# wuxiaolang/Cube_SLAM_wu

Hardware: AMD Instinct MI355X
Metric: frames/sec detect_cuboid (higher is better)
Workload: dtype f64

## Files before the change

### cube_slam_wu_amd/csrc/detect_host.cpp

```cpp
#include <hip/hip_runtime.h>

#include <algorithm>
#include <atomic>
#include <condition_variable>
#include <memory>
#include <mutex>
#include <chrono>
#include <cmath>
#include <limits>
#include <cstdio>
#include <cstring>
#include <functional>
#include <numeric>
#include <string>
#include <thread>
#include <vector>

#include "../../include/cubeslam_hip.h"
#include "detect_types.h"

namespace cs {
void launch_vp_support(const DetectDeviceView& v, const SweepParams& sp, int vp_total, hipStream_t st);
void launch_vp_support_only(const DetectDeviceView& v, const SweepParams& sp, int vp_total, hipStream_t st, int rp_max = 0);
void launch_vp_points(const DetectDeviceView& v, int vp_total, hipStream_t st);
// ... 289 lines not shown
    std::iota(keep.begin(), keep.end(), 0);
  }
  int k = (int)keep.size();
  double dmin = 1e6, dmax = -1, amin = 1e6, amax = -1;
  for (int i = 0; i < k; i++) {
    double d = dist[keep[i]], a = angle[keep[i]];
    dmin = std::min(dmin, d); dmax = std::max(dmax, d);
    amin = std::min(amin, a); amax = std::max(amax, a);
  }
  score.resize(k);
  if (k > 1) {
    bool na = (amax - amin) > 0;
    for (int i = 0; i < k; i++) {
      double d = (dist[keep[i]] - dmin) / (dmax - dmin);
      double a = angle[keep[i]];
      if (na) a = (a - amin) / (amax - amin);
      score[i] = (d + w_angle * a) / (1 + w_angle);
    }
  } else {
    for (int i = 0; i < k; i++) score[i] = (dist[keep[i]] + w_angle * angle[keep[i]]) / (1 + w_angle);
  }
}

}

struct cs_detector {
  cs_detect_params prm;
  int device = 0;
  hipStream_t stream = nullptr;
  hipStream_t stream2 = nullptr;
  hipStream_t stream3 = nullptr;
  hipStream_t stream4 = nullptr;
  hipStream_t stream_hi = nullptr;
  hipEvent_t ev[12] = {};
  int n_threads = 1;
  int cpu_grant = 1;
  std::unique_ptr<WorkerPool> pool;
  cs_batch* single = nullptr;
  std::mutex single_mu;
  void* lines_scratch = nullptr;
  void (*lines_free)(void*) = nullptr;
  void* lsd_scratch = nullptr;
  void (*lsd_free)(void*) = nullptr;
  std::mutex lines_mu;
};

struct FrameIn {
  double K[9], invK[9], R[9], t[3];
  int img_w, img_h, n_boxes, n_lines;
  std::vector<double> boxes;
  std::vector<double> lines;
  std::vector<long long> map_offs;
  std::vector<cs_roi> rois;
  std::vector<int> n_heights;
};

struct JobHost {
  int frame, box, hid;
  int yaw_off_local;
  std::vector<double> mids_x, mids_y, angs;
  std::vector<int> tops;
  int line_cap = 0;
};

struct FrameRound {
  std::vector<cs::JobDesc> jobs;
  std::vector<JobHost> jh;
  std::vector<double> yaw, yaw_c, yaw_s;
// ... 33 lines not shown
  DevBuf<unsigned long long> rp_pool_used;
  DevBuf<double> rp_raw_euler;
  PinBuf<int> h_rp_tab_count, h_rp_maps;
  PinBuf<double> h_rp_raw_euler;
  PinBuf<long long> h_rp_last_slot, h_rp_box_base;
  PinBuf<unsigned long long> h_rp_pool_used;
  long long rp_pool_cap = 0;
  int rp_NT = 0, rp_YCAP = 0;
  std::vector<hipEvent_t> rp_ev;
  bool rp_mode = false;
  PinBuf<cs::JobDesc> h_jobs_in, h_jobs_out;
  PinBuf<long long> h_slot_prefix, h_job_cbase;
  PinBuf<int> h_vp_prefix, h_top_x, h_box_job0, h_box_njobs, h_win_count, h_fallback, h_job_valid;
  PinBuf<double> h_yaw, h_yaw_c, h_yaw_s;
  PinBuf<long long> h_fb_src, h_fb_dst, h_fb_slot, h_win_slots;
  PinBuf<int> h_fb_cnt, h_fb_flag;
  PinBuf<double> h_fb_dist, h_fb_angle, h_fb_skew, h_win_corners;
  hipEvent_t done = nullptr, ev[13] = {};
  cs::DetectDeviceView view{};
  int f0 = 0, f1 = 0, vp_total = 0;
  size_t nj = 0, nb = 0;
  long long slot_total = 0;
  bool in_flight = false;
  void release() {
    jobs.release(); slot_prefix.release(); job_cbase.release(); c_slot.release(); fb_slot.release();
    vp_prefix.release(); top_x.release(); flag.release(); job_valid.release(); c_flag.release(); box_job0.release(); box_njobs.release(); win_count.release();
    fallback.release(); fb_flag.release(); mid_x.release(); mid_y.release(); ang.release(); yaw.release(); yaw_c.release(); yaw_s.release();
    vp.release(); bound.release(); bound3.release(); ls_order.release(); blk_info.release(); ls_crowded.release(); h_ls_order.release(); c_dist.release(); c_angle.release(); c_skew.release(); fb_dist.release(); fb_angle.release(); fb_skew.release();
    winners.release(); records.release(); h_records.release(); rp_trip_cnt.release(); rp_cur_idx.release(); rp_tab_count.release(); rp_maps.release(); rp_last_slot.release(); rp_box_base.release(); rp_pool_used.release(); rp_raw_euler.release(); h_rp_tab_count.release(); h_rp_maps.release(); h_rp_raw_euler.release(); h_rp_last_slot.release(); h_rp_box_base.release(); h_rp_pool_used.release(); h_jobs_in.release(); h_jobs_out.release(); h_slot_prefix.release(); h_job_cbase.release(); h_vp_prefix.release();
    h_top_x.release(); h_box_job0.release(); h_box_njobs.release(); h_win_count.release(); h_fallback.release(); h_job_valid.release(); h_yaw.release();
    h_yaw_c.release(); h_yaw_s.release();
    h_fb_src.release(); h_fb_dst.release(); h_fb_slot.release(); h_win_slots.release(); h_fb_cnt.release(); h_fb_flag.release(); h_fb_dist.release(); h_fb_angle.release();
    h_fb_skew.release(); h_win_corners.release();
    if (done) (void)hipEventDestroy(done);
    for (auto& e : ev) if (e) (void)hipEventDestroy(e);
    for (auto& e : rp_ev) if (e) (void)hipEventDestroy(e);
    rp_ev.clear();
    done = nullptr; for (auto& e : ev) e = nullptr;
  }
};

struct BatchRunState;
struct cs_batch {
  cs_detector* det = nullptr;
  BatchRunState* run_state = nullptr;
  PinBuf<cs::RpPose> h_rp;
// ... 126 lines not shown
void** cs_internal_detector_lines_slot(cs_detector* d, void (*deleter)(void*)) { d->lines_free = deleter; return &d->lines_scratch; }
void** cs_internal_detector_lsd_slot(cs_detector* d, void (*deleter)(void*)) { d->lsd_free = deleter; return &d->lsd_scratch; }
void* cs_internal_detector_lines_mutex(cs_detector* d) { return (void*)&d->lines_mu; }
void cs_internal_detector_parallel(cs_detector* d, int n, void (*fn)(int, void*), void* ctx) { d->pool->run(n, [&](int i) { fn(i, ctx); }); }
void cs_internal_detector_parallel_long(cs_detector* d, int n, void (*fn)(int, void*), void* ctx) { d->pool->run(n, [&](int i) { fn(i, ctx); }, 2 * d->cpu_grant + 1); }
int cs_internal_detector_device(cs_detector* d) { return d->device; }

int cs_detector_create(const cs_detect_params* params, int device, cs_detector** out) {
  if (!out) return CS_ERR_INVALID_ARG;
  *out = nullptr;
  int n = 0;
  if (hipGetDeviceCount(&n) != hipSuccess || n <= 0) {
    set_err("no HIP device visible; libcubeslam_hip has no CPU fallback");
    return CS_ERR_NO_DEVICE;
  }
  if (device < 0 || device >= n) { set_err("device index out of range"); return CS_ERR_INVALID_ARG; }
  CS_GUARD_BEGIN
  struct Guard { cs_detector* d; ~Guard() { if (d) cs_detector_destroy(d); } } g{new cs_detector()};
  cs_detector* d = g.d;
  if (params) d->prm = *params; else cs_detect_default_params(&d->prm);
  if (d->prm.max_cuboid_num < 1 || !(d->prm.yaw_step_deg > 0) || !(d->prm.yaw_range_deg >= 0)) { set_err("bad params"); return CS_ERR_INVALID_ARG; }
  d->device = device;
  HIP_TRY(hipSetDevice(device));
  HIP_TRY(hipStreamCreateWithFlags(&d->stream, hipStreamNonBlocking));
  HIP_TRY(hipStreamCreateWithFlags(&d->stream2, hipStreamNonBlocking));
  HIP_TRY(hipStreamCreateWithFlags(&d->stream3, hipStreamNonBlocking));
  HIP_TRY(hipStreamCreateWithFlags(&d->stream4, hipStreamNonBlocking));
  {
    int prio_low = 0, prio_high = 0;
    HIP_TRY(hipDeviceGetStreamPriorityRange(&prio_low, &prio_high));
    HIP_TRY(hipStreamCreateWithPriority(&d->stream_hi, hipStreamNonBlocking, prio_high));
  }
  for (auto& e : d->ev) HIP_TRY(hipEventCreate(&e));
  int hc = (int)std::thread::hardware_concurrency();
  int dflt = std::max(1, std::min(hc, 64));
  d->cpu_grant = std::max(1, hc);
  if (FILE* fq = std::fopen("/sys/fs/cgroup/cpu.max", "r")) {
    long long quota = 0, period = 0;
    if (std::fscanf(fq, "%lld %lld", &quota, &period) == 2 && quota > 0 && period > 0) {
      dflt = std::max(1, std::min(dflt, std::max(8, (int)(3 * quota / period))));
      d->cpu_grant = std::max(1, std::min(d->cpu_grant, (int)(quota / period)));
    }
    std::fclose(fq);
  }
  d->n_threads = d->prm.host_threads > 0 ? d->prm.host_threads : dflt;
  d->pool.reset(new WorkerPool(d->n_threads - 1));
  *out = d;
  g.d = nullptr;
  return CS_OK;
  CS_GUARD_END("cs_detector_create")
}

void cs_detector_destroy(cs_detector* d) {
  if (!d) return;
  (void)hipSetDevice(d->device);
  if (d->single) { cs_batch_destroy(d->single); d->single = nullptr; }
  if (d->lines_scratch && d->lines_free) { d->lines_free(d->lines_scratch); d->lines_scratch = nullptr; }
  if (d->lsd_scratch && d->lsd_free) { d->lsd_free(d->lsd_scratch); d->lsd_scratch = nullptr; }
  for (auto& e : d->ev) if (e) (void)hipEventDestroy(e);
  if (d->stream) (void)hipStreamDestroy(d->stream);
  if (d->stream2) (void)hipStreamDestroy(d->stream2);
  if (d->stream3) (void)hipStreamDestroy(d->stream3);
  if (d->stream4) (void)hipStreamDestroy(d->stream4);
  if (d->stream_hi) (void)hipStreamDestroy(d->stream_hi);
  delete d;
}

static int batch_fill(cs_detector* d, cs_batch* b, const cs_frame_desc* fr, const unsigned char* const* grays, int n_frames);
static void edge_rois_largest_first(std::vector<cs::EdgeRoi>& er) {
  if (er.size() <= 1024) return;
  std::stable_sort(er.begin(), er.end(), [](const cs::EdgeRoi& a, const cs::EdgeRoi& c) { return (long long)a.w * a.h > (long long)c.w * c.h; });
}
static int batch_layout(cs_detector* d, cs_batch* b);
static int batch_run_impl(cs_detector* d, cs_batch* b, cs_cuboid* out, int* out_counts, bool defer);
static int batch_flush_refill(cs_detector* d, cs_batch* b);
static void release_batch_buffers(cs_batch* b);
static int batch_create_impl(cs_detector* d, const cs_frame_desc* fr, const unsigned char* const* grays, int n_frames, cs_batch** out) {
  if (!d || !out || (!fr && n_frames) || n_frames < 0) return CS_ERR_INVALID_ARG;
  *out = nullptr;
  CS_GUARD_BEGIN
  HIP_TRY(hipSetDevice(d->device));
  struct Guard { cs_batch* b; ~Guard() { if (b) cs_batch_destroy(b); } } g{new cs_batch()};
  g.b->det = d;
  int rc = batch_fill(d, g.b, fr, grays, n_frames);
  if (rc) return rc;
  *out = g.b;
  g.b = nullptr;
// ... 192 lines not shown
    cs::launch_edge_maps(nxt ? b->d_gray2.p : b->d_gray.p, b->gray_w, b->gray_h, b->d_edge_rois.p, b->edge_n_rois, b->d_cls.p, b->d_maps.p, b->edge_max_w, b->edge_max_px, 80, 200, st);
    HIP_TRY(hipGetLastError());
  }
  HIP_TRY(hipEventRecord(b->ev_edge_done[nxt], st));
  b->gray_cur = nxt;
  b->refill_q[0] = b->refill_q[1]; b->refill_q[1] = -1; b->n_refill--;
  return CS_OK;
}
int cs_batch_refill_wait(cs_batch* b) {
  if (!b) return CS_ERR_INVALID_ARG;
  if (!b->copy_stream) return CS_OK;
  HIP_TRY(hipSetDevice(b->det->device));
  HIP_TRY(hipStreamSynchronize(b->copy_stream));
  return CS_OK;
}

int cs_batch_max_boxes(const cs_batch* b) { return b ? b->max_boxes : CS_ERR_INVALID_ARG; }

static void batch_drop_run_state(cs_batch* b);
void cs_batch_destroy(cs_batch* b) {
  if (!b) return;
  (void)hipSetDevice(b->det->device);
  if (b->run_state) { (void)hipDeviceSynchronize(); batch_drop_run_state(b); }
  release_batch_buffers(b);
  delete b;
}
static void release_batch_buffers(cs_batch* b) {
  b->pipe[0].release(); b->pipe[1].release();
  b->d_maps.release(); b->d_invK.release(); b->d_frame_lines.release(); b->d_frame_line_ptr.release(); b->d_jobs.release(); b->d_slot_prefix.release(); b->d_job_cbase.release();
  b->d_c_slot.release(); b->d_win_slots.release(); b->d_vp_prefix.release(); b->d_top_x.release(); b->d_flag.release();
  b->d_job_valid.release(); b->d_c_flag.release(); b->d_mid_x.release(); b->d_mid_y.release(); b->d_ang.release();
  b->d_yaw.release(); b->d_yaw_c.release(); b->d_yaw_s.release(); b->d_vp.release(); b->d_bound.release(); b->d_dist.release();
  b->d_angle.release(); b->d_skew.release(); b->d_corners.release(); b->d_c_dist.release(); b->d_c_angle.release();
  b->d_c_skew.release(); b->d_win_corners.release(); b->d_rp.release(); b->h_rp.release();
  b->d_gray.release(); b->d_cls.release(); b->d_edge_rois.release(); b->h_maps_stage.release(); b->d_gray2.release();
  if (b->copy_stream) { (void)hipStreamSynchronize(b->copy_stream); (void)hipStreamDestroy(b->copy_stream); b->copy_stream = nullptr; }
  for (auto& e : b->ev_copied) if (e) { (void)hipEventDestroy(e); e = nullptr; }
  for (auto& e : b->ev_edge_done) if (e) { (void)hipEventDestroy(e); e = nullptr; }
  b->h_stage.release(); b->h_c_slot.release(); b->h_job_cbase.release(); b->h_c_flag.release(); b->h_job_valid.release();
  b->h_c_dist.release(); b->h_c_angle.release(); b->h_c_skew.release(); b->h_win_corners.release();
  b->d_box_job0.release(); b->d_box_njobs.release(); b->d_win_count.release(); b->d_fallback.release(); b->d_winners.release(); b->d_last_slot.release(); b->h_last_slot.release();
  b->h_winners.release(); b->h_win_count.release(); b->h_fallback.release(); b->h_jobs.release(); b->h_tables.release(); b->h_tables2.release();
  b->d_fb_src.release(); b->d_fb_dst.release(); b->d_fb_slot.release(); b->d_fb_cnt.release(); b->d_fb_flag.release();
  b->d_fb_dist.release(); b->d_fb_angle.release(); b->d_fb_skew.release();
}

// ... 181 lines not shown
      for (int q = 0; q < NBK; q++) cnt[q + 1] += cnt[q];
      for (size_t j = 0; j < nj; j++) S.h_ls_order.p[cnt[bucket(S.h_jobs_in.p[j])]++] = (int)j;
    }
    if (vo > 0x7fffffffLL) { set_err("too many yaw samples in one chunk"); return CS_ERR_CAPACITY; }
  }
  S.nb = nb;
  MARK(1, tq);
  MARK(2, tq);
  C.tm->setup_host_ms += now_ms() - t0;
  C.tm->n_jobs += (long long)nj; C.tm->n_slots += real_slots;
  const long long slot_total = S.slot_total;
  PENS(S.ls_order, nj); PENS(S.jobs, nj); PENS(S.slot_prefix, nj + 1); PENS(S.vp_prefix, nj + 1); PENS(S.job_valid, nj); PENS(S.job_cbase, nj + 1);
  PENS(S.mid_x, n_lines + 1); PENS(S.mid_y, n_lines + 1); PENS(S.ang, n_lines + 1); PENS(S.yaw, n_yaw + 1); PENS(S.yaw_c, n_yaw + 1); PENS(S.yaw_s, n_yaw + 1);
  PENS(S.top_x, n_top + 1); PENS(S.vp, 6 * (size_t)S.vp_total + 6); PENS(S.bound, 6 * (size_t)S.vp_total + 6); PENS(S.bound3, nj * (size_t)cs::vp3_table_doubles_per_job());
  PENS(S.blk_info, 2 * (size_t)(slot_total >> 8) + 4); PENS(S.ls_crowded, 2 * (nj + 1) + 2);
  PENS(S.c_slot, slot_total + 1); PENS(S.c_flag, slot_total + 1); PENS(S.c_dist, slot_total + 1);
  PENS(S.c_angle, slot_total + 1); PENS(S.c_skew, slot_total + 1); PENS(S.box_job0, nb + 1); PENS(S.box_njobs, nb + 1); PENS(S.win_count, nb + 1);
  PENS(S.fallback, nb + 1); PENS(S.winners, nb * KMAX + 1); PENS(S.records, nb * KMAX + 1); PENS(S.h_records, nb * KMAX + 1);
  PENS(S.h_win_count, nb + 1); PENS(S.h_fallback, nb + 1); PENS(S.h_job_valid, nj); PENS(S.h_job_cbase, nj + 1); PENS(S.h_jobs_out, nj);
  int* p_ls_order = S.ls_order.p; cs::JobDesc* p_jobs = S.jobs.p; long long* p_slot_prefix = S.slot_prefix.p; int* p_vp_prefix = S.vp_prefix.p;
  double *p_yaw = S.yaw.p, *p_yaw_c = S.yaw_c.p, *p_yaw_s = S.yaw_s.p;
  int *p_top_x = S.top_x.p, *p_box_job0 = S.box_job0.p, *p_box_njobs = S.box_njobs.p;
  cs_cuboid* p_records = S.records.p; int *p_win_count = S.win_count.p, *p_fallback = S.fallback.p, *p_job_valid = S.job_valid.p; long long* p_job_cbase = S.job_cbase.p;
  S.merged_io = nj <= 256;
  if (S.merged_io) {
    size_t need = 0;
    auto room = [&](size_t bytes) { const size_t at = need; need += (bytes + 255) & ~(size_t)255; return at; };
    const size_t o_ls = room(sizeof(int) * nj), o_sp = room(sizeof(long long) * (nj + 1)), o_vp = room(sizeof(int) * (nj + 1));
    const size_t o_y = room(8 * n_yaw), o_yc = room(8 * n_yaw), o_ys = room(8 * n_yaw), o_tx = room(sizeof(int) * n_top), o_b0 = room(sizeof(int) * nb), o_bn = room(sizeof(int) * nb);
    const size_t o_jobs = room(sizeof(cs::JobDesc) * nj), in_end = need;
    S.o_jobs = o_jobs; S.o_rec = room(sizeof(cs_cuboid) * nb * KMAX); S.o_wc = room(sizeof(int) * nb); S.o_fb = room(sizeof(int) * nb); S.o_jv = room(sizeof(int) * nj);
    S.o_cb = room(sizeof(long long) * (nj + 1)); S.o_end = need;
    PENS(S.tab_arena, need + 256); PENS(S.h_tab_arena, need + 256);
    unsigned char *hb = S.h_tab_arena.p, *db = S.tab_arena.p;
    memcpy(hb + o_ls, S.h_ls_order.p, sizeof(int) * nj); memcpy(hb + o_jobs, S.h_jobs_in.p, sizeof(cs::JobDesc) * nj);
    memcpy(hb + o_sp, S.h_slot_prefix.p, sizeof(long long) * (nj + 1)); memcpy(hb + o_vp, S.h_vp_prefix.p, sizeof(int) * (nj + 1));
    if (n_yaw) { memcpy(hb + o_y, S.h_yaw.p, 8 * n_yaw); memcpy(hb + o_yc, S.h_yaw_c.p, 8 * n_yaw); memcpy(hb + o_ys, S.h_yaw_s.p, 8 * n_yaw); }
    if (n_top) memcpy(hb + o_tx, S.h_top_x.p, sizeof(int) * n_top);
    if (nb) { memcpy(hb + o_b0, S.h_box_job0.p, sizeof(int) * nb); memcpy(hb + o_bn, S.h_box_njobs.p, sizeof(int) * nb); }
    HIP_TRY(hipMemcpyAsync(db, hb, in_end, hipMemcpyHostToDevice, st));
    p_ls_order = reinterpret_cast<int*>(db + o_ls); p_jobs = reinterpret_cast<cs::JobDesc*>(db + o_jobs); p_slot_prefix = reinterpret_cast<long long*>(db + o_sp);
    p_vp_prefix = reinterpret_cast<int*>(db + o_vp); p_yaw = reinterpret_cast<double*>(db + o_y); p_yaw_c = reinterpret_cast<double*>(db + o_yc); p_yaw_s = reinterpret_cast<double*>(db + o_ys);
    p_top_x = reinterpret_cast<int*>(db + o_tx); p_box_job0 = reinterpret_cast<int*>(db + o_b0); p_box_njobs = reinterpret_cast<int*>(db + o_bn);
    p_records = reinterpret_cast<cs_cuboid*>(db + S.o_rec); p_win_count = reinterpret_cast<int*>(db + S.o_wc); p_fallback = reinterpret_cast<int*>(db + S.o_fb);
    p_job_valid = reinterpret_cast<int*>(db + S.o_jv); p_job_cbase = reinterpret_cast<long long*>(db + S.o_cb);
  } else {
    cs::CopySegs cp{};
    cs::add_copy(cp, S.ls_order, S.h_ls_order, nj); cs::add_copy(cp, S.jobs, S.h_jobs_in, nj); cs::add_copy(cp, S.slot_prefix, S.h_slot_prefix, nj + 1);
    cs::add_copy(cp, S.vp_prefix, S.h_vp_prefix, nj + 1); cs::add_copy(cp, S.yaw, S.h_yaw, n_yaw); cs::add_copy(cp, S.yaw_c, S.h_yaw_c, n_yaw);
    cs::add_copy(cp, S.yaw_s, S.h_yaw_s, n_yaw); cs::add_copy(cp, S.top_x, S.h_top_x, n_top); cs::add_copy(cp, S.box_job0, S.h_box_job0, nb);
    cs::add_copy(cp, S.box_njobs, S.h_box_njobs, nb);
    cs::launch_multi_copy(cp, st);
  }
  cs::DetectDeviceView& v = S.view;
  v = cs::DetectDeviceView{};
  v.jobs = p_jobs; v.n_jobs = (int)nj; v.slot_prefix = p_slot_prefix; v.vp_prefix = p_vp_prefix; v.maps = b->d_maps.p;
  v.mid_x = S.mid_x.p; v.mid_y = S.mid_y.p; v.line_angle = S.ang.p; v.yaw = p_yaw; v.yaw_cos = p_yaw_c; v.yaw_sin = p_yaw_s; v.top_x = p_top_x;
  v.rp = b->d_rp.p; v.invK = b->d_invK.p; v.vp = S.vp.p; v.bound = S.bound.p; v.bound3 = S.bound3.p; v.job_valid = p_job_valid;
  v.job_cbase = p_job_cbase; v.c_slot = S.c_slot.p; v.c_flag = S.c_flag.p; v.c_dist = S.c_dist.p; v.c_angle = S.c_angle.p; v.c_skew = S.c_skew.p;
  hipStream_t stB = d->stream2;
  HIP_TRY(hipEventRecord(S.ev[7], st));
  HIP_TRY(hipStreamWaitEvent(stB, S.ev[7], 0));
  HIP_TRY(hipEventRecord(S.ev[8], stB));
  v.blk_info = S.blk_info.p;
  HIP_TRY(hipMemsetAsync(S.blk_info.p, 0, sizeof(int), stB));
  cs::launch_candidate_compact(v, C.sp, stB);
  HIP_TRY(hipEventRecord(S.ev[9], stB));
  HIP_TRY(hipEventRecord(S.ev[10], stB));
  HIP_TRY(hipEventRecord(S.ev[0], st));
  cs::launch_line_setup_listed(p_jobs, (int)nj, b->d_frame_lines.p, b->d_frame_line_ptr.p, S.mid_x.p, S.mid_y.p, S.ang.p, P.pre_merge_dist_thre, P.pre_merge_angle_thre, P.edge_length_threshold, st, p_ls_order,
                               d->stream3, S.ev[0], S.ev[12], S.ls_crowded.p);
  HIP_TRY(hipEventRecord(S.ev[1], st));
  cs::launch_vp_support_only(v, C.sp, S.vp_total, st, 1);
  HIP_TRY(hipEventRecord(S.ev[2], st));
  HIP_TRY(hipStreamWaitEvent(st, S.ev[10], 0));
  HIP_TRY(hipEventRecord(S.ev[4], st));
  cs::launch_score(v, C.sp, slot_total, slot_total, st);
  HIP_TRY(hipEventRecord(S.ev[5], st));
  cs::RankView rv{};
  rv.box_job0 = p_box_job0; rv.box_njobs = p_box_njobs; rv.n_boxes = (int)nb; rv.winners = S.winners.p; rv.win_count = p_win_count; rv.fallback = p_fallback;
  cs::RankParams rkp{P.weight_vp_angle, P.weight_skew_error, P.nominal_skew_ratio, P.max_cut_skew, KMAX, C.sp.short_sq_bound};
  cs::launch_rank(v, rv, rkp, st, 0, false);
  cs::launch_records(v, rv, KMAX, p_records, st, nullptr, rkp.short_sq_bound);
  HIP_TRY(hipEventRecord(S.ev[6], st));
  HIP_TRY(hipGetLastError());
  if (S.merged_io) {
    HIP_TRY(hipMemcpyAsync(S.h_tab_arena.p + S.o_jobs, S.tab_arena.p + S.o_jobs, S.o_end - S.o_jobs, hipMemcpyDeviceToHost, st));
  } else {
    cs::CopySegs cp{};
    cs::add_copy(cp, S.h_records, S.records, nb * KMAX); cs::add_copy(cp, S.h_win_count, S.win_count, nb); cs::add_copy(cp, S.h_fallback, S.fallback, nb);
    cs::add_copy(cp, S.h_job_valid, S.job_valid, nj); cs::add_copy(cp, S.h_job_cbase, S.job_cbase, nj + 1);
    cs::launch_multi_copy(cp, st);
  }
  HIP_TRY(hipEventRecord(S.done, st));
  S.in_flight = true;
  MARK(3, tq);
  return CS_OK;
}

int pipe_finish(PipeCtx& C, PipeSlot& S, const std::vector<std::vector<CamCache>>& cam_rp) {
  cs_detector* d = C.d; cs_batch* b = C.b;
  const cs_detect_params& P = d->prm;
  const int KMAX = P.max_cuboid_num, MB = b->max_boxes;
  cs_detect_timing& tm = *C.tm;
  double tw = now_ms(), tq = tw;
  HIP_TRY(hipEventSynchronize(S.done));
  tm.d2h_ms += now_ms() - tw;
  S.in_flight = false;
  const size_t nj = S.nj, nb = S.nb;
  if (nj == 0) return CS_OK;
  if (S.merged_io) {
    const unsigned char* hb = S.h_tab_arena.p;
    memcpy(S.h_jobs_out.p, hb + S.o_jobs, sizeof(cs::JobDesc) * nj);
    if (nb) { memcpy(S.h_records.p, hb + S.o_rec, sizeof(cs_cuboid) * nb * KMAX); memcpy(S.h_win_count.p, hb + S.o_wc, sizeof(int) * nb); memcpy(S.h_fallback.p, hb + S.o_fb, sizeof(int) * nb); }
    memcpy(S.h_job_valid.p, hb + S.o_jv, sizeof(int) * nj); memcpy(S.h_job_cbase.p, hb + S.o_cb, sizeof(long long) * (nj + 1));
  }
  double t0 = now_ms();
  {
    float ms = 0;
    HIP_TRY(hipEventElapsedTime(&ms, S.ev[0], S.ev[1])); tm.line_setup_ms += ms;
    HIP_TRY(hipEventElapsedTime(&ms, S.ev[1], S.ev[2])); tm.vp_kernel_ms += ms;
    HIP_TRY(hipEventElapsedTime(&ms, S.ev[8], S.ev[9])); tm.cand_kernel_ms += ms;
    HIP_TRY(hipEventElapsedTime(&ms, S.ev[9], S.ev[10])); tm.compact_ms += ms;
    HIP_TRY(hipEventElapsedTime(&ms, S.ev[4], S.ev[5])); tm.score_kernel_ms += ms;
    HIP_TRY(hipEventElapsedTime(&ms, S.ev[5], S.ev[6])); tm.rank_kernel_ms += ms;
    tm.cand_kernel_launches += 1;
    long long n_valid = 0;
    for (size_t j = 0; j < nj; j++) n_valid += S.h_job_valid.p[j];
// ... 247 lines not shown
    slots_all += so;
  }
  const size_t nj = ji, nb = nb_tot;
  S.nj = nj; S.nb = nb; S.slot_total = slots_all; S.vp_total = vp_cap_max;
  if (n_lines > 0x7fffffffLL) { set_err("chunk too large"); return CS_ERR_CAPACITY; }
  for (size_t j = 0; j < nj; j++) S.h_ls_order.p[j] = (int)j;
  C.tm->setup_host_ms += now_ms() - t0;
  C.tm->n_jobs += (long long)nj;
  if (nj == 0) { S.in_flight = true; HIP_TRY(hipEventRecord(S.done, st)); return CS_OK; }
  PENS(S.ls_order, nj); PENS(S.jobs, nj); PENS(S.slot_prefix, nj + MB + 1); PENS(S.vp_prefix, nj + MB + 1); PENS(S.job_valid, nj); PENS(S.job_cbase, nj + MB + 1);
  const int max_trips = (int)std::min<long long>((max_job_slots + 4095) / 4096, 1 << 20);
  PENS(S.rp_trip_cnt, (size_t)nj_round_max * (size_t)std::max(1, max_trips) + 1);
  PENS(S.mid_x, (size_t)n_lines + 1); PENS(S.mid_y, (size_t)n_lines + 1); PENS(S.ang, (size_t)n_lines + 1); PENS(S.yaw, n_yaw + 1); PENS(S.yaw_c, n_yaw + 1); PENS(S.yaw_s, n_yaw + 1);
  PENS(S.top_x, n_top + 1); PENS(S.vp, 6 * (size_t)vp_cap_max + 6); PENS(S.bound, 6 * (size_t)vp_cap_max + 6); PENS(S.bound3, nj_round_max * (size_t)cs::vp3_table_doubles_per_job() + 1);
  PENS(S.flag, slot_cap_max + 1); PENS(S.c_slot, slot_cap_max + 1); PENS(S.c_flag, slot_cap_max + 1); PENS(S.c_dist, slot_cap_max + 1); PENS(S.c_angle, slot_cap_max + 1); PENS(S.c_skew, slot_cap_max + 1);
  PENS(S.box_job0, nb + 1); PENS(S.box_njobs, nb + 1); PENS(S.win_count, nb + 1); PENS(S.fallback, nb + 1); PENS(S.rp_last_slot, nb + 1);
  PENS(S.winners, nb * KMAX + 1); PENS(S.records, nb * KMAX + 1); PENS(S.h_records, nb * KMAX + 1); PENS(S.h_win_count, nb + 1); PENS(S.h_fallback, nb + 1);
  PENS(S.h_job_cbase, nj + MB + 1);
  S.rp_NT = NT; S.rp_YCAP = YCAP;
  S.rp_pool_cap = std::max<long long>(1 << 18, slots_all / 64);
  PENS(S.fb_dist, (size_t)S.rp_pool_cap + 1); PENS(S.fb_angle, (size_t)S.rp_pool_cap + 1); PENS(S.fb_skew, (size_t)S.rp_pool_cap + 1); PENS(S.fb_flag, (size_t)S.rp_pool_cap + 1); PENS(S.fb_slot, (size_t)S.rp_pool_cap + 1);
  PENS(S.ls_crowded, 2 * (nj + 1) + 2);
  PENS(S.rp_box_base, nb + 1); PENS(S.rp_pool_used, 1); PENS(S.h_rp_box_base, nb + 1); PENS(S.h_rp_pool_used, 1); PENS(S.h_rp_last_slot, nb + 1); PENS(S.h_job_valid, nj + 1); PENS(S.h_jobs_out, nj + 1);
  HIP_TRY(hipMemsetAsync(S.rp_pool_used.p, 0, sizeof(unsigned long long), st));
  PENS(S.rp_cur_idx, (size_t)NF + 1); PENS(S.rp_tab_count, (size_t)NF * NT + 1); PENS(S.rp_maps, 3 * (size_t)MB * NF + 1); PENS(S.rp_raw_euler, 3 * (size_t)NF + 1);
  {
    cs::CopySegs cp{};
    cs::add_copy(cp, S.ls_order, S.h_ls_order, nj); cs::add_copy(cp, S.jobs, S.h_jobs_in, nj); cs::add_copy(cp, S.slot_prefix, S.h_slot_prefix, nj + MB);
    cs::add_copy(cp, S.vp_prefix, S.h_vp_prefix, nj + MB); cs::add_copy(cp, S.yaw, S.h_yaw, n_yaw); cs::add_copy(cp, S.yaw_c, S.h_yaw_c, n_yaw);
    cs::add_copy(cp, S.yaw_s, S.h_yaw_s, n_yaw); cs::add_copy(cp, S.top_x, S.h_top_x, n_top); cs::add_copy(cp, S.box_job0, S.h_box_job0, nb);
    cs::add_copy(cp, S.box_njobs, S.h_box_njobs, nb); cs::add_copy(cp, S.rp_tab_count, S.h_rp_tab_count, (long long)NF * NT);
    cs::add_copy(cp, S.rp_maps, S.h_rp_maps, 3LL * MB * NF); cs::add_copy(cp, S.rp_raw_euler, S.h_rp_raw_euler, 3LL * NF);
    cs::launch_multi_copy(cp, st);
  }
  HIP_TRY(hipMemsetAsync(S.job_valid.p, 0, sizeof(int) * nj, st));
  HIP_TRY(hipMemsetAsync(S.rp_cur_idx.p, 0, sizeof(int) * NF, st));
  HIP_TRY(hipEventRecord(S.ev[0], st));
  cs::launch_line_setup_listed(S.jobs.p, (int)nj, b->d_frame_lines.p, b->d_frame_line_ptr.p, S.mid_x.p, S.mid_y.p, S.ang.p, P.pre_merge_dist_thre, P.pre_merge_angle_thre, P.edge_length_threshold, st, S.ls_order.p,
                               d->stream3, S.ev[0], S.ev[12], S.ls_crowded.p);
  HIP_TRY(hipEventRecord(S.ev[1], st));
  cs::RankParams rkp{P.weight_vp_angle, P.weight_skew_error, P.nominal_skew_ratio, P.max_cut_skew, KMAX, C.sp.short_sq_bound};
  while (S.rp_ev.size() < 5 * (size_t)MB) { hipEvent_t e = nullptr; HIP_TRY(hipEventCreate(&e)); S.rp_ev.push_back(e); }
  for (int r = 0; r < MB; r++) {
    const PipeSlot::RpRound& Rr = S.rp_rounds[r];
    if (Rr.nj == 0) continue;
    hipEvent_t* re = &S.rp_ev[5 * (size_t)r];
    cs::DetectDeviceView v{};
    v.jobs = S.jobs.p + Rr.j0; v.n_jobs = (int)Rr.nj; v.slot_prefix = S.slot_prefix.p + Rr.j0 + r; v.vp_prefix = S.vp_prefix.p + Rr.j0 + r; v.maps = b->d_maps.p;
    v.mid_x = S.mid_x.p; v.mid_y = S.mid_y.p; v.line_angle = S.ang.p; v.yaw = S.yaw.p; v.yaw_cos = S.yaw_c.p; v.yaw_sin = S.yaw_s.p; v.top_x = S.top_x.p;
    v.rp = b->d_rp.p; v.invK = b->d_invK.p; v.vp = S.vp.p; v.bound = S.bound.p; v.bound3 = S.bound3.p; v.flag = S.flag.p; v.job_valid = S.job_valid.p + Rr.j0;
    v.job_cbase = S.job_cbase.p + Rr.j0 + r; v.c_slot = S.c_slot.p; v.c_flag = S.c_flag.p; v.c_dist = S.c_dist.p; v.c_angle = S.c_angle.p; v.c_skew = S.c_skew.p;
    if (r > 0) {
      int rq = r - 1;
      while (rq > 0 && S.rp_rounds[rq].nj == 0) rq--;
      const PipeSlot::RpRound& Rq = S.rp_rounds[rq];
      cs::RpCarryView c{};
      c.n_frames = NF; c.NT = NT; c.YCAP = YCAP;
      c.prev_box_of_frame = Rq.nj ? S.rp_maps.p + (size_t)(3 * rq) * NF : nullptr;
      c.prev_last_slot = S.rp_last_slot.p + Rq.b0; c.prev_jobs = S.jobs.p + Rq.j0; c.prev_box_job0 = S.box_job0.p + Rq.b0; c.prev_box_njobs = S.box_njobs.p + Rq.b0;
      c.job0_of_frame = S.rp_maps.p + (size_t)(3 * r + 1) * NF; c.njobs_of_frame = S.rp_maps.p + (size_t)(3 * r + 2) * NF;
      c.tab_count = S.rp_tab_count.p; c.cur_idx = S.rp_cur_idx.p;
      cs::launch_rp_carry(c, S.jobs.p + Rr.j0, st);
    }
    HIP_TRY(hipEventRecord(re[0], st));
    cs::launch_vp_points(v, Rr.vp_cap, st);
// ... 8 lines not shown
    rv.box_job0 = S.box_job0.p + Rr.b0; rv.box_njobs = S.box_njobs.p + Rr.b0; rv.n_boxes = (int)Rr.nb; rv.winners = S.winners.p + Rr.b0 * KMAX;
    rv.win_count = S.win_count.p + Rr.b0; rv.fallback = S.fallback.p + Rr.b0; rv.last_slot = S.rp_last_slot.p + Rr.b0;
    cs::launch_rank(v, rv, rkp, st, Rr.nb ? (long long)(Rr.slot_cap / (long long)Rr.nb) : 0, false);
    cs::launch_records(v, rv, KMAX, S.records.p + Rr.b0 * KMAX, st, S.rp_raw_euler.p, rkp.short_sq_bound);
    {
      cs::RpSaveView sv{};
      sv.fallback = rv.fallback; sv.box_job0 = rv.box_job0; sv.box_njobs = rv.box_njobs; sv.n_boxes = rv.n_boxes; sv.pool_used = S.rp_pool_used.p; sv.pool_cap = S.rp_pool_cap;
      sv.box_base = S.rp_box_base.p + Rr.b0; sv.p_dist = S.fb_dist.p; sv.p_angle = S.fb_angle.p; sv.p_skew = S.fb_skew.p; sv.p_flag = S.fb_flag.p; sv.p_slot = S.fb_slot.p;
      cs::launch_rp_save_fallback(v, sv, st);
    }
    HIP_TRY(hipEventRecord(re[4], st));
    HIP_TRY(hipGetLastError());
  }
  HIP_TRY(hipEventRecord(S.ev[6], st));
  {
    cs::CopySegs cp{};
    cs::add_copy(cp, S.h_records, S.records, nb * KMAX); cs::add_copy(cp, S.h_win_count, S.win_count, nb); cs::add_copy(cp, S.h_fallback, S.fallback, nb);
    cs::add_copy(cp, S.h_job_cbase, S.job_cbase, nj + MB); cs::add_copy(cp, S.h_job_valid, S.job_valid, nj); cs::add_copy(cp, S.h_jobs_out, S.jobs, nj);
    cs::add_copy(cp, S.h_rp_last_slot, S.rp_last_slot, nb); cs::add_copy(cp, S.h_rp_box_base, S.rp_box_base, nb); cs::add_copy(cp, S.h_rp_pool_used, S.rp_pool_used, 1);
    cs::launch_multi_copy(cp, st);
  }
  HIP_TRY(hipEventRecord(S.done, st));
  S.in_flight = true;
  return CS_OK;
}

int rp_finish(PipeCtx& C, PipeSlot& S) {
  cs_detector* d = C.d; cs_batch* b = C.b;
  const cs_detect_params& P = d->prm;
  const int KMAX = P.max_cuboid_num, MB = b->max_boxes, NF = b->n_frames;
  cs_detect_timing& tm = *C.tm;
  double tw = now_ms();
  HIP_TRY(hipEventSynchronize(S.done));
  tm.d2h_ms += now_ms() - tw;
  S.in_flight = false;
  if (S.nj == 0) return CS_OK;
  double t0 = now_ms();
  {
    float ms = 0;
    HIP_TRY(hipEventElapsedTime(&ms, S.ev[0], S.ev[1])); tm.line_setup_ms += ms;
    for (int r = 0; r < MB; r++) {
      if (S.rp_rounds[r].nj == 0) continue;
      hipEvent_t* re = &S.rp_ev[5 * (size_t)r];
      HIP_TRY(hipEventElapsedTime(&ms, re[0], re[1])); tm.cand_kernel_ms += ms;
      HIP_TRY(hipEventElapsedTime(&ms, re[1], re[2])); tm.vp_kernel_ms += ms;
      HIP_TRY(hipEventElapsedTime(&ms, re[2], re[3])); tm.score_kernel_ms += ms;
      HIP_TRY(hipEventElapsedTime(&ms, re[3], re[4])); tm.rank_kernel_ms += ms;
      tm.cand_kernel_launches += 1;
    }
    tm.n_slots += S.slot_total;
    for (int r = 0; r < MB; r++) if (S.rp_rounds[r].nj) tm.n_valid += S.h_job_cbase.p[S.rp_rounds[r].j0 + r + S.rp_rounds[r].nj];
  }
  std::vector<char> redo(NF, 0);
  std::vector<char> host_done(S.nb, 0);
  int n_redo = 0;
// ... 951 lines not shown
```

### cube_slam_wu_amd/csrc/detect_kernels.hip

```cpp
#include <hip/hip_runtime.h>
#include "cs_hip_util.h"

#include <cstdio>
#include <cstdlib>
#include <cstring>

#include "../../include/cubeslam_hip.h"
#include "detect_types.h"

namespace cs {

__device__ __forceinline__ int wave_uniform_i32(int x) { return __builtin_amdgcn_readfirstlane(x); }
__device__ __forceinline__ long long wave_uniform_i64(long long x) {
  const unsigned lo = (unsigned)__builtin_amdgcn_readfirstlane((int)(unsigned)(x & 0xffffffffll)), hi = (unsigned)__builtin_amdgcn_readfirstlane((int)(x >> 32));
  return (long long)(((unsigned long long)hi << 32) | lo);
}
template <typename T>
__device__ __forceinline__ int find_job_wave(const T* __restrict__ prefix, int n, T elem) {
  const T first = sizeof(T) == 8 ? (T)wave_uniform_i64((long long)elem) : (T)wave_uniform_i32((int)elem);
  int lo = 0, hi = n;
  while (hi - lo > 1) {
    const int mid = (lo + hi) >> 1;
    if (prefix[mid] <= first) lo = mid; else hi = mid;
  }
// ... 1450 lines not shown
}
#else
static constexpr bool skip_kernel(const char*) { return false; }
#endif
void launch_line_setup(JobDesc* jobs, int n_jobs, const double* frame_lines, const int* frame_line_ptr, double* mid_x, double* mid_y, double* line_angle,
                       double dist_thre, double angle_thre_deg, double len_thre, hipStream_t st) {
  if (skip_kernel("line_setup")) return;
  if (n_jobs <= 0) return;
  LineSetupParams lp{dist_thre, angle_thre_deg / 180.0 * CS_PI, len_thre, sqrt_lt_bound(dist_thre), sqrt_le_bound(len_thre)};
  hipLaunchKernelGGL((line_setup_kernel<LS_CAP, LS_CROWDED_THREADS>), dim3(n_jobs), dim3(LS_CROWDED_THREADS), 0, st, jobs, n_jobs, frame_lines, frame_line_ptr, mid_x, mid_y, line_angle, lp, nullptr);
  hipLaunchKernelGGL(line_setup_small_kernel, dim3(n_jobs), dim3(64), 0, st, jobs, n_jobs, frame_lines, frame_line_ptr, mid_x, mid_y, line_angle, lp, nullptr);
}
void launch_line_setup_listed(JobDesc* jobs, int n_jobs, const double* frame_lines, const int* frame_line_ptr, double* mid_x, double* mid_y, double* line_angle,
                              double dist_thre, double angle_thre_deg, double len_thre, hipStream_t st, const int* order, hipStream_t st_crowded, hipEvent_t fork, hipEvent_t join, int* crowded) {
  if (skip_kernel("line_setup")) return;
  if (n_jobs <= 0) return;
  LineSetupParams lp{dist_thre, angle_thre_deg / 180.0 * CS_PI, len_thre, sqrt_lt_bound(dist_thre), sqrt_le_bound(len_thre)};
  int* big = crowded + n_jobs + 1;
  (void)hipMemsetAsync(crowded, 0, sizeof(int), st);
  (void)hipMemsetAsync(big, 0, sizeof(int), st);
  hipLaunchKernelGGL(line_classify_kernel, dim3((n_jobs + 3) / 4), dim3(256), 0, st, jobs, n_jobs, frame_lines, frame_line_ptr, crowded, big);
  (void)hipEventRecord(fork, st);
  const int grid = n_jobs < 1024 ? n_jobs : 1024;
  (void)hipStreamWaitEvent(st_crowded, fork, 0);
  hipLaunchKernelGGL((line_setup_listed_kernel<LS_CAP, LS_CROWDED_THREADS>), dim3(grid), dim3(LS_CROWDED_THREADS), 0, st_crowded, jobs, n_jobs, frame_lines, frame_line_ptr, mid_x, mid_y, line_angle, lp, big);
  hipLaunchKernelGGL((line_setup_listed_kernel<LS_MID, LS_CROWDED_THREADS>), dim3(grid), dim3(LS_CROWDED_THREADS), 0, st_crowded, jobs, n_jobs, frame_lines, frame_line_ptr, mid_x, mid_y, line_angle, lp, crowded);
  (void)hipEventRecord(join, st_crowded);
  hipLaunchKernelGGL(line_setup_small_kernel, dim3(n_jobs), dim3(64), 0, st, jobs, n_jobs, frame_lines, frame_line_ptr, mid_x, mid_y, line_angle, lp, order);
  (void)hipStreamWaitEvent(st, join, 0);
}
int line_setup_capacity() { return LS_CAP; }


template <bool REBUILD>
__global__ __launch_bounds__(64) void record_kernel(DetectDeviceView v, RankView rv, int kmax, cs_cuboid* __restrict__ out, const double* __restrict__ raw_euler, double short_sq_bound) {
  const int e = blockIdx.x * 64 + threadIdx.x;
  if (e >= rv.n_boxes * kmax) return;
  const int q = e / kmax, r = e - q * kmax;
  if (rv.fallback[q] || r >= rv.win_count[q]) return;
  const RankWinner& w = rv.winners[e];
  double wc[16];
  if (REBUILD) slot_corners16(v, w.slot, short_sq_bound, wc);
  else {
#pragma unroll
    for (int i = 0; i < 16; i++) wc[i] = w.corners[i];
  }
  const int j0 = rv.box_job0[q], nh = rv.box_njobs[q];
  int h = 0;
  while (h + 1 < nh && w.slot >= v.jobs[j0 + h + 1].slot_off) h++;
  const JobDesc& jd = v.jobs[j0 + h];
  const long long local = w.slot - jd.slot_off, rest = local >> 1;
  const int ry = (int)(rest / jd.T), rp = ry / jd.Y, y = ry - rp * jd.Y;
// ... 463 lines not shown
```

Before: 498,200.

## Share per-device stream pool across detectors mapped to hardware queues

```diff
diff --git a/cube_slam_wu_amd/csrc/detect_host.cpp b/cube_slam_wu_amd/csrc/detect_host.cpp
--- a/cube_slam_wu_amd/csrc/detect_host.cpp
+++ b/cube_slam_wu_amd/csrc/detect_host.cpp
@@ -335,15 +335,84 @@
   }
 }
 
+struct StreamSet {
+  enum { MAX_SLOTS = 16 };
+  int device = 0, refs = 0, n_queues = 4, n_slots = 0;
+  std::atomic<int> busy{0};
+  bool own_streams = false;
+  hipStream_t chain[MAX_SLOTS] = {};
+  int users[MAX_SLOTS] = {};
+  hipStream_t hi[MAX_SLOTS] = {};
+  std::mutex enqueue_mu;
+};
+std::mutex g_sets_mu;
+std::vector<StreamSet*> g_sets;
+
+int hw_queue_count() {
+  const char* e = getenv("GPU_MAX_HW_QUEUES");
+  const int n = e ? atoi(e) : 4;
+  return n < 1 ? 4 : std::min(n, 32);
+}
+
+void stream_set_destroy(StreamSet* s) {
+  for (hipStream_t st : s->chain) if (st) (void)hipStreamDestroy(st);
+  for (hipStream_t st : s->hi) if (st) (void)hipStreamDestroy(st);
+  delete s;
+}
+
+StreamSet* stream_set_acquire(int device, hipError_t* err) {
+  std::lock_guard<std::mutex> lk(g_sets_mu);
+  *err = hipSuccess;
+  for (StreamSet* s : g_sets) if (s->device == device) { s->refs++; return s; }
+  StreamSet* s = new StreamSet();
+  s->device = device; s->n_queues = hw_queue_count();
+  s->own_streams = s->n_queues >= 8;
+  s->n_slots = s->own_streams ? 0 : s->n_queues;
+  for (int i = 0; i < s->n_slots && *err == hipSuccess; i++) *err = hipStreamCreateWithFlags(&s->chain[i], hipStreamNonBlocking);
+  if (*err == hipSuccess && s->n_slots > 0) {
+    int prio_low = 0, prio_high = 0;
+    *err = hipDeviceGetStreamPriorityRange(&prio_low, &prio_high);
+    for (int i = 0; i < s->n_slots && *err == hipSuccess; i++) *err = hipStreamCreateWithPriority(&s->hi[i], hipStreamNonBlocking, prio_high);
+  }
+  if (*err != hipSuccess) { stream_set_destroy(s); return nullptr; }
+  s->refs = 1;
+  g_sets.push_back(s);
+  return s;
+}
+
+int stream_set_borrow(StreamSet* s, hipStream_t out[4]) {
+  std::lock_guard<std::mutex> lk(g_sets_mu);
+  if (s->own_streams) return -1;
+  int i = 0;
+  for (int k = 1; k < s->n_slots; k++) if (s->users[k] < s->users[i]) i = k;
+  s->users[i]++;
+  out[0] = s->chain[i];
+  out[1] = out[0];
+  out[2] = out[0];
+  out[3] = s->hi[i];
+  return i;
+}
+
+void stream_set_release(StreamSet* s, int slot) {
+  std::lock_guard<std::mutex> lk(g_sets_mu);
+  if (slot >= 0 && slot < s->n_slots) s->users[slot]--;
+  if (--s->refs > 0) return;
+  g_sets.erase(std::find(g_sets.begin(), g_sets.end(), s));
+  stream_set_destroy(s);
+}
+
 }
 
 struct cs_detector {
   cs_detect_params prm;
   int device = 0;
+  StreamSet* streams = nullptr;
+  int stream_slot = -1;
+  std::atomic<int> busy{0};
+  hipStream_t stream_idle = nullptr;
   hipStream_t stream = nullptr;
   hipStream_t stream2 = nullptr;
   hipStream_t stream3 = nullptr;
-  hipStream_t stream4 = nullptr;
   hipStream_t stream_hi = nullptr;
   hipEvent_t ev[12] = {};
   int n_threads = 1;
@@ -357,6 +426,15 @@
   void (*lsd_free)(void*) = nullptr;
   std::mutex lines_mu;
 };
+
+static void sweep_side_streams(const cs_detector* d, hipStream_t* corners, hipStream_t* crowded) {
+  const StreamSet* s = d->streams;
+  *corners = d->stream2; *crowded = d->stream3;
+  if (!s->own_streams && s->n_slots >= 3 && s->busy.load() == d->busy.load()) {
+    *corners = s->chain[(d->stream_slot + 1) % s->n_slots];
+    *crowded = s->chain[(d->stream_slot + 2) % s->n_slots];
+  }
+}
 
 struct FrameIn {
   double K[9], invK[9], R[9], t[3];
@@ -436,6 +514,7 @@
   size_t nj = 0, nb = 0;
   long long slot_total = 0;
   bool in_flight = false;
+  bool counted_busy = false;
   void release() {
     jobs.release(); slot_prefix.release(); job_cbase.release(); c_slot.release(); fb_slot.release();
     vp_prefix.release(); top_x.release(); flag.release(); job_valid.release(); c_flag.release(); box_job0.release(); box_njobs.release(); win_count.release();
@@ -608,14 +687,23 @@
   if (d->prm.max_cuboid_num < 1 || !(d->prm.yaw_step_deg > 0) || !(d->prm.yaw_range_deg >= 0)) { set_err("bad params"); return CS_ERR_INVALID_ARG; }
   d->device = device;
   HIP_TRY(hipSetDevice(device));
-  HIP_TRY(hipStreamCreateWithFlags(&d->stream, hipStreamNonBlocking));
-  HIP_TRY(hipStreamCreateWithFlags(&d->stream2, hipStreamNonBlocking));
-  HIP_TRY(hipStreamCreateWithFlags(&d->stream3, hipStreamNonBlocking));
-  HIP_TRY(hipStreamCreateWithFlags(&d->stream4, hipStreamNonBlocking));
   {
-    int prio_low = 0, prio_high = 0;
-    HIP_TRY(hipDeviceGetStreamPriorityRange(&prio_low, &prio_high));
-    HIP_TRY(hipStreamCreateWithPriority(&d->stream_hi, hipStreamNonBlocking, prio_high));
+    hipError_t se = hipSuccess;
+    d->streams = stream_set_acquire(device, &se);
+    HIP_TRY(se);
+    if (d->streams->own_streams) {
+      HIP_TRY(hipStreamCreateWithFlags(&d->stream, hipStreamNonBlocking));
+      HIP_TRY(hipStreamCreateWithFlags(&d->stream2, hipStreamNonBlocking));
+      HIP_TRY(hipStreamCreateWithFlags(&d->stream3, hipStreamNonBlocking));
+      HIP_TRY(hipStreamCreateWithFlags(&d->stream_idle, hipStreamNonBlocking));
+      int prio_low = 0, prio_high = 0;
+      HIP_TRY(hipDeviceGetStreamPriorityRange(&prio_low, &prio_high));
+      HIP_TRY(hipStreamCreateWithPriority(&d->stream_hi, hipStreamNonBlocking, prio_high));
+    } else {
+      hipStream_t st4[4];
+      d->stream_slot = stream_set_borrow(d->streams, st4);
+      d->stream = st4[0]; d->stream2 = st4[1]; d->stream3 = st4[2]; d->stream_hi = st4[3];
+    }
   }
   for (auto& e : d->ev) HIP_TRY(hipEventCreate(&e));
   int hc = (int)std::thread::hardware_concurrency();
@@ -644,11 +732,12 @@
   if (d->lines_scratch && d->lines_free) { d->lines_free(d->lines_scratch); d->lines_scratch = nullptr; }
   if (d->lsd_scratch && d->lsd_free) { d->lsd_free(d->lsd_scratch); d->lsd_scratch = nullptr; }
   for (auto& e : d->ev) if (e) (void)hipEventDestroy(e);
-  if (d->stream) (void)hipStreamDestroy(d->stream);
-  if (d->stream2) (void)hipStreamDestroy(d->stream2);
-  if (d->stream3) (void)hipStreamDestroy(d->stream3);
-  if (d->stream4) (void)hipStreamDestroy(d->stream4);
-  if (d->stream_hi) (void)hipStreamDestroy(d->stream_hi);
+  if (d->streams) {
+    if (d->stream) (void)hipStreamSynchronize(d->stream);
+    if (d->streams->own_streams)
+      for (hipStream_t st : {d->stream, d->stream2, d->stream3, d->stream_idle, d->stream_hi}) if (st) (void)hipStreamDestroy(st);
+    stream_set_release(d->streams, d->stream_slot);
+  }
   delete d;
 }
 
@@ -887,6 +976,7 @@
   if (!b) return;
   (void)hipSetDevice(b->det->device);
   if (b->run_state) { (void)hipDeviceSynchronize(); batch_drop_run_state(b); }
+  for (PipeSlot& S : b->pipe) if (S.counted_busy) { S.counted_busy = false; b->det->busy.fetch_sub(1); b->det->streams->busy.fetch_sub(1); }
   release_batch_buffers(b);
   delete b;
 }
@@ -1114,6 +1204,7 @@
   double *p_yaw = S.yaw.p, *p_yaw_c = S.yaw_c.p, *p_yaw_s = S.yaw_s.p;
   int *p_top_x = S.top_x.p, *p_box_job0 = S.box_job0.p, *p_box_njobs = S.box_njobs.p;
   cs_cuboid* p_records = S.records.p; int *p_win_count = S.win_count.p, *p_fallback = S.fallback.p, *p_job_valid = S.job_valid.p; long long* p_job_cbase = S.job_cbase.p;
+  std::unique_lock<std::mutex> enqueue(d->streams->enqueue_mu, std::defer_lock);
   S.merged_io = nj <= 256;
   if (S.merged_io) {
     size_t need = 0;
@@ -1130,6 +1221,7 @@
     if (n_yaw) { memcpy(hb + o_y, S.h_yaw.p, 8 * n_yaw); memcpy(hb + o_yc, S.h_yaw_c.p, 8 * n_yaw); memcpy(hb + o_ys, S.h_yaw_s.p, 8 * n_yaw); }
     if (n_top) memcpy(hb + o_tx, S.h_top_x.p, sizeof(int) * n_top);
     if (nb) { memcpy(hb + o_b0, S.h_box_job0.p, sizeof(int) * nb); memcpy(hb + o_bn, S.h_box_njobs.p, sizeof(int) * nb); }
+    if (!d->streams->own_streams) enqueue.lock();
     HIP_TRY(hipMemcpyAsync(db, hb, in_end, hipMemcpyHostToDevice, st));
     p_ls_order = reinterpret_cast<int*>(db + o_ls); p_jobs = reinterpret_cast<cs::JobDesc*>(db + o_jobs); p_slot_prefix = reinterpret_cast<long long*>(db + o_sp);
     p_vp_prefix = reinterpret_cast<int*>(db + o_vp); p_yaw = reinterpret_cast<double*>(db + o_y); p_yaw_c = reinterpret_cast<double*>(db + o_yc); p_yaw_s = reinterpret_cast<double*>(db + o_ys);
@@ -1142,6 +1234,7 @@
     cs::add_copy(cp, S.vp_prefix, S.h_vp_prefix, nj + 1); cs::add_copy(cp, S.yaw, S.h_yaw, n_yaw); cs::add_copy(cp, S.yaw_c, S.h_yaw_c, n_yaw);
     cs::add_copy(cp, S.yaw_s, S.h_yaw_s, n_yaw); cs::add_copy(cp, S.top_x, S.h_top_x, n_top); cs::add_copy(cp, S.box_job0, S.h_box_job0, nb);
     cs::add_copy(cp, S.box_njobs, S.h_box_njobs, nb);
+    if (!d->streams->own_streams) enqueue.lock();
     cs::launch_multi_copy(cp, st);
   }
   cs::DetectDeviceView& v = S.view;
@@ -1150,9 +1243,12 @@
   v.mid_x = S.mid_x.p; v.mid_y = S.mid_y.p; v.line_angle = S.ang.p; v.yaw = p_yaw; v.yaw_cos = p_yaw_c; v.yaw_sin = p_yaw_s; v.top_x = p_top_x;
   v.rp = b->d_rp.p; v.invK = b->d_invK.p; v.vp = S.vp.p; v.bound = S.bound.p; v.bound3 = S.bound3.p; v.job_valid = p_job_valid;
   v.job_cbase = p_job_cbase; v.c_slot = S.c_slot.p; v.c_flag = S.c_flag.p; v.c_dist = S.c_dist.p; v.c_angle = S.c_angle.p; v.c_skew = S.c_skew.p;
-  hipStream_t stB = d->stream2;
-  HIP_TRY(hipEventRecord(S.ev[7], st));
-  HIP_TRY(hipStreamWaitEvent(stB, S.ev[7], 0));
+  hipStream_t stB = nullptr, stC = nullptr;
+  sweep_side_streams(d, &stB, &stC);
+  if (stB != st) {
+    HIP_TRY(hipEventRecord(S.ev[7], st));
+    HIP_TRY(hipStreamWaitEvent(stB, S.ev[7], 0));
+  }
   HIP_TRY(hipEventRecord(S.ev[8], stB));
   v.blk_info = S.blk_info.p;
   HIP_TRY(hipMemsetAsync(S.blk_info.p, 0, sizeof(int), stB));
@@ -1161,11 +1257,11 @@
   HIP_TRY(hipEventRecord(S.ev[10], stB));
   HIP_TRY(hipEventRecord(S.ev[0], st));
   cs::launch_line_setup_listed(p_jobs, (int)nj, b->d_frame_lines.p, b->d_frame_line_ptr.p, S.mid_x.p, S.mid_y.p, S.ang.p, P.pre_merge_dist_thre, P.pre_merge_angle_thre, P.edge_length_threshold, st, p_ls_order,
-                               d->stream3, S.ev[0], S.ev[12], S.ls_crowded.p);
+                               stC, S.ev[0], S.ev[12], S.ls_crowded.p);
   HIP_TRY(hipEventRecord(S.ev[1], st));
   cs::launch_vp_support_only(v, C.sp, S.vp_total, st, 1);
   HIP_TRY(hipEventRecord(S.ev[2], st));
-  HIP_TRY(hipStreamWaitEvent(st, S.ev[10], 0));
+  if (stB != st) HIP_TRY(hipStreamWaitEvent(st, S.ev[10], 0));
   HIP_TRY(hipEventRecord(S.ev[4], st));
   cs::launch_score(v, C.sp, slot_total, slot_total, st);
   HIP_TRY(hipEventRecord(S.ev[5], st));
@@ -1186,6 +1282,7 @@
   }
   HIP_TRY(hipEventRecord(S.done, st));
   S.in_flight = true;
+  S.counted_busy = true; d->busy.fetch_add(1); d->streams->busy.fetch_add(1);
   MARK(3, tq);
   return CS_OK;
 }
@@ -1196,6 +1293,7 @@
   const int KMAX = P.max_cuboid_num, MB = b->max_boxes;
   cs_detect_timing& tm = *C.tm;
   double tw = now_ms(), tq = tw;
+  if (S.counted_busy) { S.counted_busy = false; d->busy.fetch_sub(1); d->streams->busy.fetch_sub(1); }
   HIP_TRY(hipEventSynchronize(S.done));
   tm.d2h_ms += now_ms() - tw;
   S.in_flight = false;
@@ -1489,8 +1587,13 @@
   PENS(S.fb_dist, (size_t)S.rp_pool_cap + 1); PENS(S.fb_angle, (size_t)S.rp_pool_cap + 1); PENS(S.fb_skew, (size_t)S.rp_pool_cap + 1); PENS(S.fb_flag, (size_t)S.rp_pool_cap + 1); PENS(S.fb_slot, (size_t)S.rp_pool_cap + 1);
   PENS(S.ls_crowded, 2 * (nj + 1) + 2);
   PENS(S.rp_box_base, nb + 1); PENS(S.rp_pool_used, 1); PENS(S.h_rp_box_base, nb + 1); PENS(S.h_rp_pool_used, 1); PENS(S.h_rp_last_slot, nb + 1); PENS(S.h_job_valid, nj + 1); PENS(S.h_jobs_out, nj + 1);
+  PENS(S.rp_cur_idx, (size_t)NF + 1); PENS(S.rp_tab_count, (size_t)NF * NT + 1); PENS(S.rp_maps, 3 * (size_t)MB * NF + 1); PENS(S.rp_raw_euler, 3 * (size_t)NF + 1);
+  while (S.rp_ev.size() < 5 * (size_t)MB) { hipEvent_t e = nullptr; HIP_TRY(hipEventCreate(&e)); S.rp_ev.push_back(e); }
+  std::unique_lock<std::mutex> enqueue(d->streams->enqueue_mu, std::defer_lock);
+  if (!d->streams->own_streams) enqueue.lock();
+  hipStream_t stB_unused = nullptr, stC = nullptr;
+  sweep_side_streams(d, &stB_unused, &stC);
   HIP_TRY(hipMemsetAsync(S.rp_pool_used.p, 0, sizeof(unsigned long long), st));
-  PENS(S.rp_cur_idx, (size_t)NF + 1); PENS(S.rp_tab_count, (size_t)NF * NT + 1); PENS(S.rp_maps, 3 * (size_t)MB * NF + 1); PENS(S.rp_raw_euler, 3 * (size_t)NF + 1);
   {
     cs::CopySegs cp{};
     cs::add_copy(cp, S.ls_order, S.h_ls_order, nj); cs::add_copy(cp, S.jobs, S.h_jobs_in, nj); cs::add_copy(cp, S.slot_prefix, S.h_slot_prefix, nj + MB);
@@ -1504,10 +1607,9 @@
   HIP_TRY(hipMemsetAsync(S.rp_cur_idx.p, 0, sizeof(int) * NF, st));
   HIP_TRY(hipEventRecord(S.ev[0], st));
   cs::launch_line_setup_listed(S.jobs.p, (int)nj, b->d_frame_lines.p, b->d_frame_line_ptr.p, S.mid_x.p, S.mid_y.p, S.ang.p, P.pre_merge_dist_thre, P.pre_merge_angle_thre, P.edge_length_threshold, st, S.ls_order.p,
-                               d->stream3, S.ev[0], S.ev[12], S.ls_crowded.p);
+                               stC, S.ev[0], S.ev[12], S.ls_crowded.p);
   HIP_TRY(hipEventRecord(S.ev[1], st));
   cs::RankParams rkp{P.weight_vp_angle, P.weight_skew_error, P.nominal_skew_ratio, P.max_cut_skew, KMAX, C.sp.short_sq_bound};
-  while (S.rp_ev.size() < 5 * (size_t)MB) { hipEvent_t e = nullptr; HIP_TRY(hipEventCreate(&e)); S.rp_ev.push_back(e); }
   for (int r = 0; r < MB; r++) {
     const PipeSlot::RpRound& Rr = S.rp_rounds[r];
     if (Rr.nj == 0) continue;
@@ -1562,6 +1664,7 @@
   }
   HIP_TRY(hipEventRecord(S.done, st));
   S.in_flight = true;
+  S.counted_busy = true; d->busy.fetch_add(1); d->streams->busy.fetch_add(1);
   return CS_OK;
 }
 
@@ -1571,6 +1674,7 @@
   const int KMAX = P.max_cuboid_num, MB = b->max_boxes, NF = b->n_frames;
   cs_detect_timing& tm = *C.tm;
   double tw = now_ms();
+  if (S.counted_busy) { S.counted_busy = false; d->busy.fetch_sub(1); d->streams->busy.fetch_sub(1); }
   HIP_TRY(hipEventSynchronize(S.done));
   tm.d2h_ms += now_ms() - tw;
   S.in_flight = false;
diff --git a/cube_slam_wu_amd/csrc/detect_kernels.hip b/cube_slam_wu_amd/csrc/detect_kernels.hip
--- a/cube_slam_wu_amd/csrc/detect_kernels.hip
+++ b/cube_slam_wu_amd/csrc/detect_kernels.hip
@@ -1496,12 +1496,12 @@
   hipLaunchKernelGGL(line_classify_kernel, dim3((n_jobs + 3) / 4), dim3(256), 0, st, jobs, n_jobs, frame_lines, frame_line_ptr, crowded, big);
   (void)hipEventRecord(fork, st);
   const int grid = n_jobs < 1024 ? n_jobs : 1024;
-  (void)hipStreamWaitEvent(st_crowded, fork, 0);
+  if (st_crowded != st) (void)hipStreamWaitEvent(st_crowded, fork, 0);
   hipLaunchKernelGGL((line_setup_listed_kernel<LS_CAP, LS_CROWDED_THREADS>), dim3(grid), dim3(LS_CROWDED_THREADS), 0, st_crowded, jobs, n_jobs, frame_lines, frame_line_ptr, mid_x, mid_y, line_angle, lp, big);
   hipLaunchKernelGGL((line_setup_listed_kernel<LS_MID, LS_CROWDED_THREADS>), dim3(grid), dim3(LS_CROWDED_THREADS), 0, st_crowded, jobs, n_jobs, frame_lines, frame_line_ptr, mid_x, mid_y, line_angle, lp, crowded);
   (void)hipEventRecord(join, st_crowded);
   hipLaunchKernelGGL(line_setup_small_kernel, dim3(n_jobs), dim3(64), 0, st, jobs, n_jobs, frame_lines, frame_line_ptr, mid_x, mid_y, line_angle, lp, order);
-  (void)hipStreamWaitEvent(st, join, 0);
+  if (st_crowded != st) (void)hipStreamWaitEvent(st, join, 0);
 }
 int line_setup_capacity() { return LS_CAP; }
 
```

New measurement: 543,500, median of 6. 9.1% higher.
